# jordisr/poreover

Hardware: AMD Instinct MI355X
Metric: decoded Mbases/s + read-pairs/s, 10k synthetic pairs T~4000, 1/2/4/8 MI355X (higher is better)
Workload: dtype f64; 1 GPU; pair-decode (Viterbi x2 + banded NW + envelope + pair beam row_col) of ONE job of 10000 synthetic pairs, T~4000, C=5, beam_width=5, padding=5; inputs resident in HBM; pairs_per_job=10000, pairs_per_gpu=10000, T=4000, beam_width=5, method=row_col, decoded_pairs_rank0=10000, parallelism=shard1 (no collective)

## Files before the change

poreover_amd/csrc/po_beam2d_pre.h:

```cpp
#pragma once
#include "po_beam2d_common.h"

template <int MODEL>
__global__ __launch_bounds__(64) void beam2d_prepass_kernel(X2Args a) {
    constexpr int K = (MODEL == PO_MODEL_CTC) ? 1 : 3;
    constexpr int nthr = 64;
    const int pi = blockIdx.x, tid = threadIdx.x;
    if (a.use_pre_status && a.status[pi] != PO_OK) {
        if (tid == 0) { a.meta[pi] = make_int2(a.status[pi], -1); a.nmain[pi] = 0; }
        return;
    }
    const int64_t o1 = a.y1_off[pi], o2 = a.y2_off[pi];
    const int64_t b2 = a.y2_off[0];
    const int U = (int)(a.y1_off[pi + 1] - o1), V = (int)(a.y2_off[pi + 1] - o2);
    const int32_t* env = a.env + 2 * o1;
    int* envt = a.envt + 2 * (o2 - b2);
    const int A = a.A, W = a.W;
    int st = PO_OK, R = 32;
    if (U < 1 || V < 1 || U >= (1 << 24) || V >= (1 << 24)) st = PO_E_ARG;
    if (st == PO_OK) {
        int bad = 0, wmax = 0, nonmono = 0;
        const int2* env2 = (const int2*)env;
        for (int u = tid; u < U; u += nthr) {
            const int2 e = env2[u];
            const int lo = e.x, hi = e.y;
            const int2 ep = (u > 0) ? env2[u - 1] : make_int2(0, 0);
            const int ln = (u + 1 < U) ? env2[u + 1].x : V;
            if (lo < hi && (lo < 0 || hi > V)) bad = 1;
            if (lo < 0 || hi > V || (u > 0 && (lo < ep.x || hi < ep.y))) nonmono = 1;
            wmax = max(wmax, hi - lo);
            const int hp = (u > 0) ? ep.y : 0;
            for (int x = max(hp, 0); x < min(hi, V); ++x) envt[2 * x] = u;
            for (int x = max(lo, 0); x < min(ln, V); ++x) envt[2 * x + 1] = u;
        }
        __threadfence_block();
        if (__syncthreads_or(bad)) st = PO_E_ENVELOPE;
        const bool mono = !__syncthreads_or(nonmono);
        if (st == PO_OK && mono) {
            const int lo0 = env[0], hil = env[2 * (U - 1) + 1];
            for (int x = tid; x < V; x += nthr) {
                const int a_ = (x < hil) ? envt[2 * x] : 0x7fffffff, b_ = (x >= lo0) ? envt[2 * x + 1] : -1;
                const int c = (a_ != 0x7fffffff && b_ >= a_) ? b_ - a_ + 1 : 0;
                envt[2 * x] = c ? a_ : -1;
                envt[2 * x + 1] = c ? a_ + c : -1;
                wmax = max(wmax, c);
            }
        } else if (st == PO_OK && !a.need_mono) {
            for (int x = tid; x < V; x += nthr) { envt[2 * x] = 0x7fffffff; envt[2 * x + 1] = 0; }
            __syncthreads();
            for (int u = tid; u < U; u += nthr) {
                const int lo = env[2 * u], hi = env[2 * u + 1];
                for (int x = lo; x < hi; ++x) { atomicMin(&envt[2 * x], u); atomicAdd(&envt[2 * x + 1], 1); }
            }
            __syncthreads();
            for (int x = tid; x < V; x += nthr) {
                const int c = envt[2 * x + 1], f = envt[2 * x];
                envt[2 * x] = c ? f : -1;
                envt[2 * x + 1] = c ? f + c : -1;
                wmax = max(wmax, c);
            }
        }
        if (st == PO_OK) {
#pragma unroll
            for (int off = 32; off >= 1; off >>= 1) wmax = max(wmax, __shfl_xor(wmax, off));
            while (R < wmax + 2) R <<= 1;
            const long long pool_entries = (long long)(a.pool_bytes / (8 * K));
            const long long ng = pool_entries / ((long long)PO_A * 2 * R);
            const long long need = 1 + A + (long long)A * max(W, A) * ((long long)min(U, V) + 1);
            if (need >= (1 << 24)) st = PO_E_NOMEM;
            else if (min((long long)a.ngl, ng) < 8 * max(W, PO_A) || ((a.defer_odd & 1) && (pi & 1)) || (a.need_mono && !mono)) R = X2_DEFERRED;
        }
    }
    if (tid == 0) {
        a.meta[pi] = make_int2(st, R);
        a.nmain[pi] = 0;
        if (st == PO_OK && R == X2_DEFERRED) {
            a.queue[16] = 1;
            if (a.defer_count) atomicAdd(a.defer_count, 1ull);
        }
    }
}

__global__ __launch_bounds__(64) void beam2d_walk_kernel(X2Args a) {
    const int pi = blockIdx.x, lane = threadIdx.x;
    const int2 mt = a.meta[pi];
    if (mt.x != PO_OK || mt.y < 0) return;
    const int64_t o1 = a.y1_off[pi], o2 = a.y2_off[pi], b2 = a.y2_off[0];
    const int U = (int)(a.y1_off[pi + 1] - o1), V = (int)(a.y2_off[pi + 1] - o2);
    const int2* env2 = (const int2*)(a.env + 2 * o1);
    const int2* envt2 = (const int2*)(a.envt + 2 * (o2 - b2));
    int4* sc = a.sched + (o2 - b2);
    int u = 0, v = 0, m = 0, werr = 0, ubase = -1000, vbase = -1000;
    int2 erc = make_int2(0, 0), ecc = make_int2(0, 0);
    while (u <= U - 1 && v <= V - 1) {
        if (u < ubase || u >= ubase + 64) { ubase = u; erc = (ubase + lane < U) ? env2[ubase + lane] : make_int2(0, 0); }
        if (v < vbase || v >= vbase + 64) { vbase = v; ecc = (vbase + lane < V) ? envt2[vbase + lane] : make_int2(0, 0); }
        const int ul = u + lane, vl = v + lane;
        const int iu = ul - ubase, iv = vl - vbase;
        const bool have = iu < 64 && iv < 64 && ul < U && vl < V;
        const int ers = __shfl(erc.x, iu & 63), ere = __shfl(erc.y, iu & 63);
        const int ecs = __shfl(ecc.x, iv & 63), ece = __shfl(ecc.y, iv & 63);
        const bool row_ok = (vl >= ers && vl < ere), col_ok = (ul >= ecs && ul < ece);
        const unsigned long long okb = __ballot(have && row_ok && col_ok);
        const unsigned long long haveb = __ballot(have);
        const int run = (~okb == 0ull) ? 64 : __builtin_ctzll(~okb);
        if (lane < run) sc[m + lane] = make_int4(ul, vl, ece, ere);
        m += run; u += run; v += run;
        if (run < 64 && ((haveb >> run) & 1ull)) {
            const unsigned long long c1 = __ballot(!row_ok && vl < ers), c0 = __ballot(!col_ok && ul < ecs);
            if ((c1 >> run) & 1ull) v = __builtin_amdgcn_readlane(ers, run);
            else if ((c0 >> run) & 1ull) {
                const int cs = __builtin_amdgcn_readlane(ecs, run);
                const int rw = u + 1 + lane, ir = rw - ubase;
                const int rws = __shfl(erc.x, ir & 63);
                const unsigned long long same = __ballot(ir < 64 && rw < cs && rw < U && !(v < rws));
                u += 1 + ((~same == 0ull) ? 64 : __builtin_ctzll(~same));
            } else { werr = 1; break; }
        }
    }
    if (lane == 0) {
        a.nmain[pi] = m;
        if (werr) a.meta[pi] = make_int2(PO_E_ENVELOPE, mt.y);
    }
}
```

poreover_amd/csrc/po_pair.hip:

```cpp
#include <algorithm>
#include <atomic>
#include <cstdlib>
#include <type_traits>

#define PO_WANT_ZERO_KERNEL 1
#include "po_device.h"
#include "po_host.h"

namespace {

constexpr int NW_MATCH = 2, NW_MISMATCH = -1, NW_GAP = -1, NW_BAND = 500;
constexpr int SK_PER = 8, SK_BW = SK_PER * 64, SK_MAXB = 256, SK_SEG = 1024;

struct PPArgs {
    const int64_t* y1_off; const int64_t* y2_off;
    int n;
    const char* seq1d; const int64_t* seq1d_off;
    const int32_t* len1; const int32_t* len2;
    const int32_t* map1; const int32_t* map2;
    const int32_t* st1; const int32_t* st2;
    int padding, full_alignment, diagonal_envelope, diagonal_width;
    int band;
    int match, mismatch, gap;
    long long seq_lds_cap;
// ... 480 lines not shown
        }
        }
        if (a.mode == 1) {
            const int64_t ao = a.aln_off[pi];
            const int capo = (int)(a.aln_off[pi + 1] - ao);
            if (ncol > capo) { if (tid == 0) { a.status[pi] = PO_E_CAP; *a.cap_flag = 1; a.ncol_out[pi] = 0; } continue; }
            for (int k = tid; k < ncol; k += NT) { a.aln_out1[ao + k] = al1[ncol - 1 - k]; a.aln_out2[ao + k] = al2[ncol - 1 - k]; }
            if (tid == 0) { a.ncol_out[pi] = ncol; a.status[pi] = PO_OK; }
            continue;
        }
        int matches = 0;
        for (int k = tid; k < ncol; k += NT) matches += (al1[k] == al2[k]);
        int tot_m;
        (void)block_excl_sum(matches, &tot_m);
        const double identity = (double)tot_m / (double)ncol;
        if (a.mode == 0 && identity < 0.5) {
            if (tid == 0) { a.status[pi] = PO_SKIP_IDENTITY; a.identity[pi] = identity; }
            continue;
        }

        PPTK(2);
        if constexpr (SKEW) if (a.maps_increasing) {
            int* const blo = r_start;
            int* const bhi = r_start + a.row_cap + 8;
            int xbase = -1, ybase = -1;
            for (int k0 = 0; k0 < ncol; k0 += PO_WAVE) {
                const int k = k0 + lane;
                const bool in = k < ncol;
                const char ca = in ? al1[ncol - 1 - k] : '-', cb = in ? al2[ncol - 1 - k] : '-';
                const char cn = (k + 1 < ncol) ? al1[ncol - 2 - k] : '-';
                int tx, ty;
                const int ex = block_excl_sum(ca != '-' ? 1 : 0, &tx);
                const int ey = block_excl_sum(cb != '-' ? 1 : 0, &ty);
                if (in) {
                    const int xi = xbase + ex + (ca != '-' ? 1 : 0);
                    const int yi = ybase + ey + (cb != '-' ? 1 : 0);
                    const int i1 = min(max(xi, 0), l1 - 1), i2 = min(max(yi, 0), l2 - 1);
                    const int i1p = min(max(xi - (ca != '-' ? 1 : 0), 0), l1 - 1);
                    const int i1n = min(max(xi + (cn != '-' ? 1 : 0), 0), l1 - 1);
                    if (k == 0 || i1p != i1) blo[i1] = m2[i2];
                    if (k == ncol - 1 || i1n != i1) bhi[i1] = (i2 + 1 < l2) ? m2[i2 + 1] : V;
                }
                xbase += tx;
                ybase += ty;
            }
            psync();
            {
                const int f0 = min(m1[0], U);
                int lo = 0, hi = min(V, -1 + a.padding);
                if (lo > hi) lo = 0;
                for (int u = lane; u < f0; u += PO_WAVE) { env[2 * u] = lo; env[2 * u + 1] = hi; }
            }
            int pe_ = 0;
            for (int b0 = 0; b0 < l1; b0 += PO_WAVE) {
                const int b = b0 + lane;
                const bool in = b < l1;
                int lo = 0, hi = 0, r0 = 0, r1 = 0;
                if (in) {
                    lo = max(0, blo[b] - a.padding);
                    hi = min(V, bhi[b] + a.padding);
                    if (lo > hi) lo = 0;
                    r0 = m1[b];
                    r1 = min((b + 1 < l1) ? m1[b + 1] : U, U);
                }
                int lo_first = lo, pos = 0;
                for (;;) {
                    const unsigned long long mk = __ballot(in && r0 < r1 && lane >= pos && lo_first > pe_);
                    if (mk == 0ull) break;
                    const int qs = __builtin_ctzll(mk);
                    if (lane == qs) lo_first = pe_;
                    pe_ = __builtin_amdgcn_readlane(hi, qs);
                    pos = qs + 1;
                }
                for (int u = r0; u < r1; ++u) { env[2 * u] = (u == r0) ? lo_first : lo; env[2 * u + 1] = hi; }
            }
            if (tid == 0) { a.status[pi] = PO_OK; if (a.identity) a.identity[pi] = identity; }
            PPTK(3);
#ifdef PO_PP_TIMING
            if (tid == 0 && pi == 0) printf("[pp timing] pair 0: setup %lld fill %lld traceback %lld envelope %lld ticks (10 ns)\n", tk_[0], tk_[1], tk_[2], tk_[3]);
#endif
            continue;
        }
        for (int u = tid; u < U; u += NT) { env[2 * u] = INT_MAX; env[2 * u + 1] = -1; }
        __syncthreads();
        int xbase = -1, ybase = -1;
        for (int k0 = 0; k0 < ncol; k0 += NT) {
            const int k = k0 + tid;
            const bool in = k < ncol;
            const char ca = in ? al1[ncol - 1 - k] : '-', cb = in ? al2[ncol - 1 - k] : '-';
            int tx, ty;
            const int ex = block_excl_sum(ca != '-' ? 1 : 0, &tx);
            const int ey = block_excl_sum(cb != '-' ? 1 : 0, &ty);
            if (in) {
                const int xi = xbase + ex + (ca != '-' ? 1 : 0);
                const int yi = ybase + ey + (cb != '-' ? 1 : 0);
                const int i1 = min(max(xi, 0), l1 - 1), i2 = min(max(yi, 0), l2 - 1);
                const int sx = m1[i1], exr = (i1 + 1 < l1) ? m1[i1 + 1] : U;
                const int sy = m2[i2], eyr = (i2 + 1 < l2) ? m2[i2 + 1] : V;
                for (int i = sx; i < exr; ++i)
                    if (i < U) { atomicMin(&env[2 * i], sy); atomicMax(&env[2 * i + 1], eyr); }
            }
            xbase += tx;
            ybase += ty;
        }
        __threadfence_block();
        __syncthreads();
        int prev_end = 0;
        for (int u0 = 0; u0 < U; u0 += NT) {
            const int u = u0 + tid;
            if (u < U) {
                int lo = env[2 * u], hi = env[2 * u + 1];
                if (lo == INT_MAX) lo = -1;
                lo = max(0, lo - a.padding);
                hi = min(V, hi + a.padding);
                lo_s[tid] = lo; hi_s[tid] = hi;
            }
            __syncthreads();
            if (tid < PO_WAVE) {
                const int cnt = min(NT, U - u0);
                int pe_ = prev_end;
                for (int b0 = 0; b0 < cnt; b0 += PO_WAVE) {
                    const int q = b0 + lane;
                    const bool in = q < cnt;
                    int lo = in ? lo_s[q] : 0;
                    const int hi = in ? hi_s[q] : 0;
                    if (lo > hi) lo = 0;
                    int pos = 0;
                    for (;;) {
                        const unsigned long long mk = __ballot(in && lane >= pos && lo > pe_);
                        if (mk == 0ull) break;
                        const int qs = __builtin_ctzll(mk);
                        if (lane == qs) lo = pe_;
                        pe_ = __builtin_amdgcn_readlane(hi, qs);
                        pos = qs + 1;
                    }
                    if (in) lo_s[q] = lo;
                }
                if (lane == 0) sh[4] = pe_;
            }
            __syncthreads();
            prev_end = sh[4];
            if (u < U) { env[2 * u] = lo_s[tid]; env[2 * u + 1] = hi_s[tid]; }
            __syncthreads();
        }
        if (tid == 0) { a.status[pi] = PO_OK; if (a.identity) a.identity[pi] = identity; }
        PPTK(3);
#ifdef PO_PP_TIMING
        if (tid == 0 && pi == 0) printf("[pp timing] pair 0: setup %lld fill %lld traceback %lld envelope %lld ticks (10 ns)\n", tk_[0], tk_[1], tk_[2], tk_[3]);
#endif
    }
}

extern "C" {
int po_launch_viterbi_strided(const double*, const int64_t*, int, int, int, uint32_t, int, int8_t*, char*,
                              const int64_t*, int, int, int32_t*, int32_t*, int32_t*, int8_t*, int8_t*, hipStream_t);
size_t po_beam2d_ws_bytes_impl(int, int64_t, int64_t, int64_t, int64_t, int, int, int, int);
int po_launch_beam2d_geom(const double*, const int64_t*, const double*, const int64_t*, const int32_t*, int, int, int,
                          uint32_t, int, int, int, int64_t, int64_t, int64_t, int64_t, char*, const int64_t*, int32_t*, int32_t*,
                          int, void*, size_t, hipStream_t);
void po_prof_stage(int kernel, hipStream_t s, int begin, void** tok);
}

static std::atomic<int> g_pp_legacy{-1};
extern "C" int po_set_align_route(int legacy) {
    g_pp_legacy.store(legacy ? 1 : 0);
    return PO_OK;
}
static bool pp_legacy() {
    int v = g_pp_legacy.load();
    if (v < 0) {
        const char* e = getenv("PO_PP_LEGACY");
        v = (e != nullptr && atoi(e) != 0) ? 1 : 0;
        g_pp_legacy.store(v);
    }
    return v != 0;
}

namespace {
void pp_launch(PPArgs a, int blocks, int one_wave, hipStream_t stream, long long max_len2 = 0) {
    long long cap = (a.mode == 2) ? 0 : ((a.row_cap + 15) & ~15LL);
    if (cap > 24 * 1024) cap = 0;
    a.seq_lds_cap = cap;
    const size_t lds = (size_t)(2 * cap);
    const bool legacy = pp_legacy();
    const bool skew = one_wave && !a.full_alignment && a.mode != 2 && !legacy && max_len2 <= (long long)SK_MAXB * SK_BW;
    if (skew) hipLaunchKernelGGL((pair_prep_kernel<64, true>), dim3(blocks), dim3(64), lds, stream, a);
    else if (one_wave) hipLaunchKernelGGL((pair_prep_kernel<64, false>), dim3(blocks), dim3(64), lds, stream, a);
    else hipLaunchKernelGGL((pair_prep_kernel<256, false>), dim3(blocks), dim3(256), lds, stream, a);
}
}

namespace {
inline size_t al256(size_t b) { return (b + 255) & ~size_t(255); }

inline size_t pp_skew_cells(int64_t l1, int64_t l2, int64_t band) {
    const int64_t nb = l2 / SK_BW + 1;
    const int64_t rows = 2 * (l1 + 1) + ((l1 + 1) * (2 * band + 1) + l2) / SK_BW + 1 + nb;
    return (size_t)(64 * (rows + 63 * nb));
}

struct PPGeom {
    int blocks, one_wave;
    size_t dp_cap, row_cap, aln_cap;
    int big_blocks;
    size_t big_dp_cap, big_row_cap, big_aln_cap, off_big_dp, off_big_rows, off_big_aln;
    size_t off_queue, off_map1, off_map2, off_st1, off_st2, off_dp, off_rows, off_aln, off_ff, off_env, off_b2, total;
    size_t ff_bytes, b2_bytes;
};

size_t pp_total_mem() { return po_dev_info().mem; }

int pp_num_cus() { return po_dev_info().cus; }

PPGeom pp_geometry(int n, int64_t tr1, int64_t tr2, int64_t mr1, int64_t mr2, int C, const po_pair_options* opt) {
    PPGeom g;
    g.one_wave = opt->full_alignment ? 0 : 1;
    g.blocks = std::min(n > 0 ? n : 1, pp_num_cus() * (g.one_wave ? 16 : 4));
    const int64_t lmax1 = std::max<int64_t>(64, mr1 / 4 + 8), lmax2 = std::max<int64_t>(64, mr2 / 4 + 8);
    g.row_cap = (size_t)(lmax1 + 1);
    const int64_t width = opt->full_alignment ? (lmax2 + 1) : std::min<int64_t>(lmax2 + 1, 2 * NW_BAND + 1);
    const bool skew_only = g.one_wave && !pp_legacy() && lmax2 <= (int64_t)SK_MAXB * SK_BW && mr2 + 8 <= (int64_t)SK_MAXB * SK_BW;
    g.dp_cap = skew_only ? pp_skew_cells(lmax1, lmax2, NW_BAND) : (size_t)((lmax1 + 1) * width);
    if (g.one_wave && !skew_only) g.dp_cap = std::max(g.dp_cap, pp_skew_cells(lmax1, lmax2, NW_BAND));
    g.aln_cap = (size_t)(lmax1 + lmax2 + 16);
    {
        static const size_t budget = [] { const char* e = getenv("PO_PP_BUDGET_MB"); return (size_t)(e ? atoi(e) : 5120) << 20; }();
        const size_t per_block = sizeof(int) * g.dp_cap + sizeof(int) * 4 * g.row_cap + 2 * g.aln_cap;
        const size_t pb = std::max<size_t>(per_block, 1);
        const size_t fit_budget = std::max<size_t>(budget / pb, (size_t)pp_num_cus());
        const size_t fit_mem = std::max<size_t>(1, (pp_total_mem() / 16) / pb);
        g.blocks = (int)std::min<size_t>((size_t)g.blocks, std::max<size_t>(1, std::min(fit_budget, fit_mem)));
    }
    {
        const int64_t b1 = mr1 + 8, b2 = mr2 + 8;
        g.big_row_cap = (size_t)(b1 + 1);
        const int64_t bw = opt->full_alignment ? (b2 + 1) : std::min<int64_t>(b2 + 1, 2 * NW_BAND + 1);
        g.big_dp_cap = skew_only ? pp_skew_cells(b1, b2, NW_BAND) : (size_t)((b1 + 1) * bw);
        if (g.one_wave && !skew_only) g.big_dp_cap = std::max(g.big_dp_cap, pp_skew_cells(b1, b2, NW_BAND));
        g.big_aln_cap = (size_t)(b1 + b2 + 16);
        const size_t per_block = sizeof(int) * g.big_dp_cap + sizeof(int) * 4 * g.big_row_cap + 2 * g.big_aln_cap;
        const size_t fit = ((size_t)2 << 30) / std::max<size_t>(per_block, 1);
        g.big_blocks = (int)std::max<size_t>(1, std::min<size_t>(std::min<size_t>(32, fit), (size_t)(n > 0 ? n : 1)));
        if (per_block > pp_total_mem() / 8) g.big_blocks = 0;
    }
    const int kind = opt->model == PO_MODEL_FLIPFLOP ? PO_KIND_FLIPFLOP : PO_KIND_POREOVER;
    g.ff_bytes = (kind == PO_KIND_FLIPFLOP) ? al256((size_t)std::max(tr1, tr2) * 8) + al256((size_t)std::max(tr1, tr2)) : 0;
    g.b2_bytes = po_beam2d_ws_bytes_impl(n, tr1, tr2, mr1, mr2, C, opt->beam_width, opt->model, opt->method);
    size_t o = 0;
    g.off_queue = o; o += 256;
    g.off_map1 = o; o += al256(sizeof(int32_t) * (size_t)tr1);
    g.off_map2 = o; o += al256(sizeof(int32_t) * (size_t)tr2);
    g.off_st1 = o; o += al256(sizeof(int32_t) * (size_t)n);
    g.off_st2 = o; o += al256(sizeof(int32_t) * (size_t)n);
    g.off_dp = o; o += al256(sizeof(int) * g.dp_cap * g.blocks);
    g.off_rows = o; o += al256(sizeof(int) * 4 * g.row_cap * g.blocks);
    g.off_aln = o; o += al256(2 * g.aln_cap * g.blocks);
    g.off_big_dp = o; o += al256(sizeof(int) * g.big_dp_cap * g.big_blocks);
    g.off_big_rows = o; o += al256(sizeof(int) * 4 * g.big_row_cap * g.big_blocks);
    g.off_big_aln = o; o += al256(2 * g.big_aln_cap * g.big_blocks);
    g.off_ff = o; o += g.ff_bytes;
    g.off_env = o; o += al256(sizeof(int32_t) * 2 * (size_t)tr1);
    g.off_b2 = o; o += g.b2_bytes;
    g.total = o + 256;
    return g;
}
}

extern "C" size_t po_pair_ws_bytes_impl(int n, int64_t tr1, int64_t tr2, int64_t mr1, int64_t mr2, int C,
                                        const po_pair_options* opt) {
    return pp_geometry(n, tr1, tr2, mr1, mr2, C, opt).total;
}

extern "C" int po_launch_pair_decode_geom(const double* y1, const int64_t* y1_off, const double* y2,
                                          const int64_t* y2_off, int n, int C, const po_pair_options* opt,
                                          int64_t tr1, int64_t tr2, int64_t mr1, int64_t mr2,
                                          const int32_t* ext_map1, const int32_t* ext_map2, char* seq1d,
                                          const int64_t* seq1d_off, int32_t* len1, int32_t* len2, double* identity,
                                          int32_t* env_out, char* seq, const int64_t* seq_off, int32_t* seq_len,
                                          int32_t* status, void* ws, size_t ws_bytes, hipStream_t stream) {
    if (n <= 0) return PO_OK;
    const int A = PO_A;
    const uint32_t alphabet = 'A' | ('C' << 8) | ('G' << 16) | ((uint32_t)'T' << 24);
    if (opt->model < 0 || opt->model > 2) return PO_E_ARG;
    if ((opt->model == PO_MODEL_FLIPFLOP) ? (C != 2 * A) : (C != A + 1)) return PO_E_ARG;
    const int kind = opt->model == PO_MODEL_CTC ? PO_KIND_POREOVER
                                                 : (opt->model == PO_MODEL_MERGE ? PO_KIND_BONITO : PO_KIND_FLIPFLOP);
    const PPGeom g = pp_geometry(n, tr1, tr2, mr1, mr2, C, opt);
    if (ws_bytes < g.total) return PO_E_CAP;
    char* w = (char*)ws;
    int32_t* map1 = (int32_t*)(w + g.off_map1);
    int32_t* map2 = (int32_t*)(w + g.off_map2);
    int32_t* st1 = (int32_t*)(w + g.off_st1);
    int32_t* st2 = (int32_t*)(w + g.off_st2);
    int32_t* env = env_out ? env_out : (int32_t*)(w + g.off_env);
    int8_t* ffp = g.ff_bytes ? (int8_t*)(w + g.off_ff) : nullptr;
    int8_t* ffpath = ffp ? ffp + al256((size_t)std::max(tr1, tr2) * 8) : nullptr;
    void* tok = nullptr;
    int rc;
    if (ext_map1 && ext_map2) {
        map1 = const_cast<int32_t*>(ext_map1);
        map2 = const_cast<int32_t*>(ext_map2);
        if (po_zero_async(st1, sizeof(int32_t) * n, stream) != hipSuccess) return PO_E_HIP;
        if (po_zero_async(st2, sizeof(int32_t) * n, stream) != hipSuccess) return PO_E_HIP;
    } else if (!opt->diagonal_envelope) {
        po_prof_stage(PO_K_VITERBI, stream, 1, &tok);
        rc = po_launch_viterbi_strided(y1, y1_off, n, C, A, alphabet, kind, nullptr, seq1d, seq1d_off, 0, 2, len1, map1,
                                       st1, ffp, ffpath, stream);
        if (rc != PO_OK) return rc;
        rc = po_launch_viterbi_strided(y2, y2_off, n, C, A, alphabet, kind, nullptr, seq1d, seq1d_off, 1, 2, len2, map2,
                                       st2, ffp, ffpath, stream);
        if (rc != PO_OK) return rc;
        po_prof_stage(PO_K_VITERBI, stream, 0, &tok);
    } else {
        if (po_zero_async(len1, sizeof(int32_t) * n, stream) != hipSuccess) return PO_E_HIP;
        if (po_zero_async(len2, sizeof(int32_t) * n, stream) != hipSuccess) return PO_E_HIP;
    }
    PPArgs a;
    a.y1_off = y1_off; a.y2_off = y2_off; a.n = n;
    a.seq1d = seq1d; a.seq1d_off = seq1d_off; a.len1 = len1; a.len2 = len2;
    a.map1 = map1; a.map2 = map2; a.st1 = st1; a.st2 = st2;
    a.padding = opt->padding; a.full_alignment = opt->full_alignment;
    a.diagonal_envelope = opt->diagonal_envelope; a.diagonal_width = opt->diagonal_width;
    a.band = NW_BAND; a.mode = 0; a.retry_cap = 0;
    a.maps_increasing = (ext_map1 && ext_map2) ? 0 : 1;
    a.match = NW_MATCH; a.mismatch = NW_MISMATCH; a.gap = NW_GAP;
    a.lenU = a.lenV = nullptr; a.map1_off = a.map2_off = nullptr; a.aln_out1 = a.aln_out2 = nullptr;
    a.aln_off = nullptr; a.ncol_out = nullptr; a.env_off = nullptr;
    a.env = env; a.identity = identity; a.status = status;
    a.queue = (int*)(w + g.off_queue);
    a.cap_flag = a.queue + 32;
    a.dp = (int*)(w + g.off_dp); a.dp_cap = (long long)g.dp_cap;
    a.rowinfo = (int*)(w + g.off_rows); a.row_cap = (long long)g.row_cap;
    a.aln = w + g.off_aln; a.aln_cap = (long long)g.aln_cap;
    if (po_zero_async(a.queue, 256, stream) != hipSuccess) return PO_E_HIP;
    po_prof_stage(PO_K_ALIGN, stream, 1, &tok);
    pp_launch(a, g.blocks, g.one_wave, stream, mr2 + 8);
    if (g.big_blocks > 0 && !opt->diagonal_envelope) {
        PPArgs b = a;
        b.retry_cap = 1;
        b.queue = a.queue + 16;
        b.dp = (int*)(w + g.off_big_dp); b.dp_cap = (long long)g.big_dp_cap;
        b.rowinfo = (int*)(w + g.off_big_rows); b.row_cap = (long long)g.big_row_cap;
        b.aln = w + g.off_big_aln; b.aln_cap = (long long)g.big_aln_cap;
        pp_launch(b, g.big_blocks, g.one_wave, stream, mr2 + 8);
    }
    po_prof_stage(PO_K_ALIGN, stream, 0, &tok);
    po_prof_stage(PO_K_BEAM2D, stream, 1, &tok);
    rc = po_launch_beam2d_geom(y1, y1_off, y2, y2_off, env, n, C, A, alphabet, opt->beam_width, opt->model, opt->method,
                               tr1, tr2, mr1, mr2, seq, seq_off, seq_len, status, 1, w + g.off_b2, g.b2_bytes, stream);
    po_prof_stage(PO_K_BEAM2D, stream, 0, &tok);
    return rc;
}

extern "C" int po_launch_pair_decode(const double* y1, const int64_t* y1_off, const double* y2, const int64_t* y2_off,
                                     int n, int C, const po_pair_options* opt, char* seq1d, const int64_t* seq1d_off,
                                     int32_t* len1, int32_t* len2, double* identity, int32_t* env_out, char* seq,
                                     const int64_t* seq_off, int32_t* seq_len, int32_t* status, void* ws,
                                     size_t ws_bytes, hipStream_t stream) {
    if (n <= 0) return PO_OK;
    int64_t* h = (int64_t*)malloc(sizeof(int64_t) * 2 * (size_t)(n + 1));
    if (!h) return PO_E_NOMEM;
    int rc = PO_OK;
    if (hipMemcpyAsync(h, y1_off, sizeof(int64_t) * (n + 1), hipMemcpyDeviceToHost, stream) != hipSuccess ||
        hipMemcpyAsync(h + n + 1, y2_off, sizeof(int64_t) * (n + 1), hipMemcpyDeviceToHost, stream) != hipSuccess ||
        hipStreamSynchronize(stream) != hipSuccess)
        rc = PO_E_HIP;
    int64_t m1 = 0, m2 = 0, t1 = 0, t2 = 0;
    if (rc == PO_OK) {
        for (int i = 0; i < n; ++i) {
            m1 = std::max<int64_t>(m1, h[i + 1] - h[i]);
            m2 = std::max<int64_t>(m2, h[n + 1 + i + 1] - h[n + 1 + i]);
        }
        t1 = h[n] - h[0];
        t2 = h[2 * n + 1] - h[n + 1];
    }
    free(h);
    if (rc != PO_OK) return rc;
    return po_launch_pair_decode_geom(y1, y1_off, y2, y2_off, n, C, opt, t1, t2, m1, m2, nullptr, nullptr, seq1d, seq1d_off, len1, len2,
                                      identity, env_out, seq, seq_off, seq_len, status, ws, ws_bytes, stream);
}

extern "C" size_t po_align_ws_bytes(int n, int64_t max_len1, int64_t max_len2, int band) {
    const int blocks = std::min(n > 0 ? n : 1, pp_num_cus() * 4);
    const int64_t width = band > 0 ? std::min<int64_t>(max_len2 + 1, 2 * (int64_t)band + 1) : max_len2 + 1;
    size_t cells = (size_t)((max_len1 + 1) * width);
    if (band > 0) cells = std::max(cells, pp_skew_cells(max_len1, max_len2, band));
    return 256 + al256(sizeof(int) * cells * blocks) + al256(sizeof(int) * 4 * (size_t)(max_len1 + 2) * blocks) +
           al256(2 * (size_t)(max_len1 + max_len2 + 16) * blocks) + 256;
}

extern "C" int po_launch_align_scores(const char* seqs, const int64_t* seq_off, int n, int band, int match, int mismatch,
                                      int gap, int64_t max_len1, int64_t max_len2, char* aln1, char* aln2,
                                      const int64_t* aln_off, int32_t* ncol, int32_t* status, void* ws, size_t ws_bytes,
                                      hipStream_t stream);
extern "C" int po_launch_align(const char* seqs, const int64_t* seq_off, int n, int band, int64_t max_len1,
                               int64_t max_len2, char* aln1, char* aln2, const int64_t* aln_off, int32_t* ncol,
                               int32_t* status, void* ws, size_t ws_bytes, hipStream_t stream) {
    return po_launch_align_scores(seqs, seq_off, n, band, NW_MATCH, NW_MISMATCH, NW_GAP, max_len1, max_len2, aln1, aln2, aln_off,
                                  ncol, status, ws, ws_bytes, stream);
}
extern "C" int po_launch_align_scores(const char* seqs, const int64_t* seq_off, int n, int band, int match, int mismatch,
                                      int gap, int64_t max_len1, int64_t max_len2, char* aln1, char* aln2,
                                      const int64_t* aln_off, int32_t* ncol, int32_t* status, void* ws, size_t ws_bytes,
                                      hipStream_t stream) {
    if (n <= 0) return PO_OK;
    if (ws_bytes < po_align_ws_bytes(n, max_len1, max_len2, band)) return PO_E_CAP;
    const int blocks = std::min(n, pp_num_cus() * 4);
    const int64_t width = band > 0 ? std::min<int64_t>(max_len2 + 1, 2 * (int64_t)band + 1) : max_len2 + 1;
    char* w = (char*)ws;
    const int one_wave = band > 0 ? 1 : 0;
    PPArgs a = {};
    a.n = n; a.seq1d = seqs; a.seq1d_off = seq_off; a.mode = 1;
    a.full_alignment = band > 0 ? 0 : 1; a.band = band > 0 ? band : 0;
    a.match = match; a.mismatch = mismatch; a.gap = gap;
    a.aln_out1 = aln1; a.aln_out2 = aln2; a.aln_off = aln_off; a.ncol_out = ncol; a.status = status;
    size_t o = 0;
    a.queue = (int*)(w + o); o += 256;
    a.cap_flag = a.queue + 32;
    a.dp_cap = (long long)((max_len1 + 1) * width);
    if (band > 0) a.dp_cap = std::max<long long>(a.dp_cap, (long long)pp_skew_cells(max_len1, max_len2, band));
    a.dp = (int*)(w + o); o += al256(sizeof(int) * (size_t)a.dp_cap * blocks);
    a.row_cap = (long long)(max_len1 + 2); a.rowinfo = (int*)(w + o); o += al256(sizeof(int) * 4 * (size_t)a.row_cap * blocks);
    a.aln_cap = (long long)(max_len1 + max_len2 + 16); a.aln = w + o;
    if (po_zero_async(a.queue, 256, stream) != hipSuccess) return PO_E_HIP;
    pp_launch(a, blocks, one_wave, stream, max_len2);
    return PO_OK;
}

__global__ __launch_bounds__(64) void nw_matrix_kernel(const char* seqs, const int64_t* seq_off, int n, int match, int mismatch, int gap,
                                                       int32_t* dp, const int64_t* dp_off, int32_t* status) {
    const int p = (int)blockIdx.x, lane = (int)threadIdx.x;
    if (p >= n) return;
    const char* const s1 = seqs + seq_off[2 * p];
    const char* const s2 = seqs + seq_off[2 * p + 1];
    const int l1 = (int)(seq_off[2 * p + 1] - seq_off[2 * p]), l2 = (int)(seq_off[2 * p + 2] - seq_off[2 * p + 1]);
    int32_t* const M = dp + dp_off[p];
    const int64_t Wd = (int64_t)l2 + 1;
    for (int j = lane; j <= l2; j += 64) M[j] = gap * j;
    for (int i = 1; i <= l1; ++i) {
        po_wave_sync();
        const int32_t* const up_ = M + (int64_t)(i - 1) * Wd;
        int32_t* const row = M + (int64_t)i * Wd;
        const char ci = s1[i - 1];
        int carry = gap * i;
        if (lane == 0) row[0] = carry;
        for (int base = 1; base <= l2; base += 64) {
            const int j = base + lane;
            const bool ok = j <= l2;
            int v = INT_MIN / 2;
            if (ok) {
                const int sc = (ci == s2[j - 1]) ? match : mismatch;
                v = max(up_[j - 1] + sc, up_[j] + gap) - gap * j;
            }
#pragma unroll
            for (int d = 1; d < 64; d <<= 1) {
                const int o = __shfl_up(v, d);
                if (lane >= d) v = max(v, o);
            }
            v = max(v, carry);
            if (ok) row[j] = v + gap * j;
            carry = __shfl(v, 63);
        }
    }
// ... 52 lines not shown
```

poreover_amd/csrc/po_viterbi.hip:

```cpp
#include <cstdlib>

#include "po_device.h"

#define VT_THREADS 256
#define VT_WAVES (VT_THREADS / PO_WAVE)

__device__ __forceinline__ int block_exclusive_count(bool flag, int* wsum, int* total) {
    const unsigned long long mask = __ballot(flag);
    const int lane = po_lane(), wave = threadIdx.x >> 6;
    const int below = __popcll(mask & ((1ull << lane) - 1ull));
    if (lane == 0) wsum[wave] = __popcll(mask);
    __syncthreads();
    int base = 0, tot = 0;
#pragma unroll
    for (int w = 0; w < VT_WAVES; ++w) {
        const int c = wsum[w];
        if (w < wave) base += c;
        tot += c;
    }
    __syncthreads();
    *total = tot;
    return base + below;
}

#define VT_FPT 2
#define VT_CMAX (PO_A + 1)
template <int THREADS>
__global__ __launch_bounds__(THREADS) void viterbi_ctc_kernel(
    const double* __restrict__ y, const int64_t* __restrict__ y_off, int C, uint32_t alphabet, int kind,
    int8_t* __restrict__ path, char* __restrict__ seq, const int64_t* __restrict__ seq_off, int so_base,
    int so_stride, int32_t* __restrict__ seq_len, int32_t* __restrict__ map, int32_t* __restrict__ status) {
    constexpr int VT_WAVES_ = THREADS / PO_WAVE, VT_TILE = THREADS * VT_FPT, VT_LD = (VT_TILE * VT_CMAX) / THREADS;
    __shared__ double tile[VT_TILE * VT_CMAX];
    __shared__ int wsum[VT_WAVES_];
    __shared__ int8_t pth[VT_TILE + 1];
    const int r = blockIdx.x, tid = threadIdx.x;
    const int64_t r0 = y_off[r];
    const int T = (int)(y_off[r + 1] - r0);
    const int blank = C - 1;
    const double* yr = y + r0 * C;
    const int64_t so = seq_off[so_base + (int64_t)r * so_stride];
    char* sq = seq + so;
    const int cap = (int)(seq_off[so_base + (int64_t)r * so_stride + 1] - so);
    int32_t* mp = map ? map + r0 : nullptr;
    int n_seq = 0, n_map = 0, st = PO_OK;

    int last_state = -1;
    if (kind == PO_KIND_BONITO && T > 0) {
        const double* row = yr + (int64_t)(T - 1) * C;
        int b = 0;
        double bv = row[0];
        for (int c = 1; c < C; ++c) {
            const double v = row[c];
            if (v > bv) { bv = v; b = c; }
        }
        last_state = b;
    }
    if (tid == 0) pth[0] = -1;
    __syncthreads();

    for (int t0 = 0; t0 < T; t0 += VT_TILE) {
        const int rows = min(VT_TILE, T - t0);
        const int nval = rows * C;
        const double* src = yr + (int64_t)t0 * C;
        double2 reg[VT_LD / 2];
        const double2* src2 = (const double2*)src;
        const int nval2 = nval >> 1;
#pragma unroll
        for (int q = 0; q < VT_LD / 2; ++q) {
            const int i = tid + q * THREADS;
            reg[q] = (i < nval2) ? src2[i] : make_double2(0.0, 0.0);
        }
        const double tail = (nval & 1) ? src[nval - 1] : 0.0;
#pragma unroll
        for (int q = 0; q < VT_LD / 2; ++q) {
            const int i = tid + q * THREADS;
            if (i < nval2) { tile[2 * i] = reg[q].x; tile[2 * i + 1] = reg[q].y; }
        }
        if ((nval & 1) && tid == 0) tile[nval - 1] = tail;
        __syncthreads();
        int p[VT_FPT];
#pragma unroll
        for (int f = 0; f < VT_FPT; ++f) {
            const int fr = tid * VT_FPT + f;
            p[f] = blank;
            if (fr < rows) {
                double bv = tile[fr * C];
                int b = 0;
                for (int c = 1; c < C; ++c) {
                    const double v = tile[fr * C + c];
                    if (v > bv) { bv = v; b = c; }
                }
                p[f] = b;
                pth[fr + 1] = (int8_t)b;
                if (path) path[r0 + t0 + fr] = (int8_t)b;
            }
        }
        __syncthreads();
        bool emit[VT_FPT], emit_map[VT_FPT];
        int ne = 0, nm = 0;
#pragma unroll
        for (int f = 0; f < VT_FPT; ++f) {
            const int fr = tid * VT_FPT + f, t = t0 + fr;
            const int prev = pth[fr];
            emit[f] = emit_map[f] = false;
            if (fr < rows && p[f] != blank) {
                if (kind == PO_KIND_POREOVER) {
                    emit[f] = emit_map[f] = true;
                } else {
                    emit[f] = (t == 0) || (p[f] != prev);
                    emit_map[f] = (p[f] != ((t == 0) ? last_state : prev));
                }
            }
            ne += emit[f];
            nm += emit_map[f];
        }
        auto block_excl = [&](int v, int* total) {
            const int lane = po_lane(), wave = tid >> 6;
            int inc = v;
#pragma unroll
            for (int o = 1; o < PO_WAVE; o <<= 1) {
                const int t = __shfl_up(inc, o);
                if (lane >= o) inc += t;
            }
            if (lane == PO_WAVE - 1) wsum[wave] = inc;
            __syncthreads();
            int base = 0, tot = 0;
#pragma unroll
            for (int w = 0; w < VT_WAVES_; ++w) {
                const int c = wsum[w];
                if (w < wave) base += c;
                tot += c;
            }
            __syncthreads();
            *total = tot;
            return base + inc - v;
        };
        int tot_p;
        const int excl = block_excl(ne | (nm << 16), &tot_p);
        int pos_s = n_seq + (excl & 0xffff);
#pragma unroll
        for (int f = 0; f < VT_FPT; ++f)
            if (emit[f]) {
                if (pos_s < cap) sq[pos_s] = (char)((alphabet >> (8 * p[f])) & 0xffu);
                else st = PO_E_CAP;
                pos_s++;
            }
        n_seq += tot_p & 0xffff;
        if (mp) {
            int pos_m = n_map + (excl >> 16);
#pragma unroll
            for (int f = 0; f < VT_FPT; ++f)
                if (emit_map[f]) mp[pos_m++] = t0 + tid * VT_FPT + f;
            n_map += tot_p >> 16;
        }
        if (tid == 0) pth[0] = pth[rows];
        __syncthreads();
    }
    if (__syncthreads_or(st != PO_OK)) st = PO_E_CAP;
    if (st == PO_OK && mp && n_map != n_seq) st = PO_E_ARG;
    if (T < 1) st = PO_E_ARG;
    if (tid == 0) {
        seq_len[r] = n_seq;
        status[r] = st;
    }
}

#define FF_S 8
__global__ __launch_bounds__(PO_WAVE) void flipflop_dp_kernel(const double* __restrict__ y,
                                                              const int64_t* __restrict__ y_off, int n, int A,
                                                              int8_t* __restrict__ ptr,
                                                              int8_t* __restrict__ path,
                                                              int32_t* __restrict__ status) {
    __shared__ __attribute__((aligned(8))) int8_t chunk[8][512 * FF_S];
    const int lane = po_lane(), g = lane >> 3, j = lane & 7;
    const int r = blockIdx.x * 8 + g;
    const bool live = r < n;
    const int64_t r0 = live ? y_off[r] : 0;
    const int T = live ? (int)(y_off[r + 1] - r0) : 0;
    int Tmax = T;
#pragma unroll
    for (int o = 8; o < PO_WAVE; o <<= 1) Tmax = max(Tmax, __shfl_xor(Tmax, o));
    const int S = 2 * A;
    const double* yr = y + r0 * S;
    int8_t* pr = ptr + r0 * FF_S;
    double v = (T > 0 && j < S) ? yr[j] : PO_NEG_INF;
    constexpr int FF_PF = 16;
    auto row_at = [&](int t) -> double { return (t < T && j < S) ? yr[(int64_t)t * S + j] : 0.0; };
    double yq[FF_PF];
    int bq[FF_PF];
#pragma unroll
    for (int i = 0; i < FF_PF; ++i) { yq[i] = row_at(1 + i); bq[i] = -1; }
    for (int t0 = 1; t0 < Tmax + FF_PF; t0 += FF_PF) {
#pragma unroll
        for (int i = 0; i < FF_PF; ++i) po_settle(yq[i]);
        double yn[FF_PF];
#pragma unroll
        for (int i = 0; i < FF_PF; ++i) yn[i] = row_at(t0 + FF_PF + i);
#pragma unroll
        for (int i = 0; i < FF_PF; ++i)
            if (bq[i] >= 0) pr[(int64_t)(t0 - FF_PF + i) * FF_S + j] = (int8_t)bq[i];
#pragma unroll
        for (int f = 0; f < FF_PF; ++f) {
            const int t = t0 + f;
            bq[f] = -1;
            if (t < Tmax) {
                const bool on = t < T;
                const double yt = yq[f];
                double bv = 0;
                int bi = 0;
#pragma unroll
                for (int i = 0; i < FF_S; ++i) {
                    const double vi = __shfl(v, (g << 3) | i);
                    const double tr = (j < A) ? 1.0 : (((i % A) == (j - A)) ? 1.0 : 0.0);
                    const double cand = tr + vi;
                    if (i < S && (i == 0 || cand > bv)) { bv = cand; bi = i; }
                }
                if (on && j < S) {
                    bq[f] = bi;
                    v = yt + bv;
                }
            }
        }
#pragma unroll
        for (int i = 0; i < FF_PF; ++i) yq[i] = yn[i];
    }
    double bv = __shfl(v, g << 3);
    int best = 0;
#pragma unroll
    for (int i = 1; i < FF_S; ++i) {
        const double vi = __shfl(v, (g << 3) | i);
        if (i < S && vi > bv) { bv = vi; best = i; }
    }
    __threadfence_block();
    int cur = best;
    for (int lo = ((Tmax + 511) / 512 - 1) * 512; lo >= 0; lo -= 512) {
        const int hi = min(T, lo + 512), len = hi - lo;
        {
            const unsigned long long* src = (const unsigned long long*)(pr + (int64_t)lo * FF_S);
            unsigned long long* dst = (unsigned long long*)&chunk[g][0];
            if (((unsigned long long)src & 7ull) == 0ull) {
                for (int f = j; f < len; f += 8) dst[f] = src[f];
            } else {
                for (int i = j; i < len * FF_S; i += 8) chunk[g][i] = pr[(int64_t)lo * FF_S + i];
            }
        }
        __syncthreads();
        if (j == 0) {
            for (int t = hi - 1; t >= lo; --t) {
                path[r0 + t] = (int8_t)cur;
                if (t > 0) cur = chunk[g][(t - lo) * FF_S + cur];
            }
        }
        cur = __shfl(cur, g << 3);
        __syncthreads();
    }
    if (live && j == 0) status[r] = (T < 1) ? PO_E_ARG : PO_OK;
}

__global__ __launch_bounds__(VT_THREADS) void flipflop_compact_kernel(
    const int8_t* __restrict__ path, const int64_t* __restrict__ y_off, int A, uint32_t alphabet,
    char* __restrict__ seq, const int64_t* __restrict__ seq_off, int so_base, int so_stride,
    int32_t* __restrict__ seq_len, int32_t* __restrict__ map, int32_t* __restrict__ status) {
    __shared__ int wsum[VT_WAVES];
    const int r = blockIdx.x, tid = threadIdx.x;
    const int64_t r0 = y_off[r];
    const int T = (int)(y_off[r + 1] - r0);
    const int64_t so = seq_off[so_base + (int64_t)r * so_stride];
    char* sq = seq + so;
    const int cap = (int)(seq_off[so_base + (int64_t)r * so_stride + 1] - so);
    int n_seq = 0, st = PO_OK;
    for (int t0 = 0; t0 < T; t0 += VT_THREADS) {
        const int t = t0 + tid;
        bool emit = false;
        int p = 0;
        if (t < T) {
            p = path[r0 + t];
            emit = (t == 0) || (p != path[r0 + t - 1]);
        }
        int tot;
        const int pos = n_seq + block_exclusive_count(emit, wsum, &tot);
        if (emit) {
            if (pos < cap) {
                sq[pos] = (char)((alphabet >> (8 * (p % A))) & 0xffu);
                if (map) map[r0 + pos] = t;
            } else st = PO_E_CAP;
        }
        n_seq += tot;
    }
    if (__syncthreads_or(st != PO_OK)) st = PO_E_CAP;
    if (tid == 0) {
        seq_len[r] = n_seq;
        if (status[r] == PO_OK) status[r] = st;
    }
}

extern "C" int po_launch_viterbi_strided(const double* y, const int64_t* y_off, int n, int C, int A,
                                         uint32_t alphabet, int kind, int8_t* path, char* seq,
                                         const int64_t* seq_off, int so_base, int so_stride, int32_t* seq_len,
                                         int32_t* map, int32_t* status, int8_t* ff_ptr, int8_t* ff_path,
                                         hipStream_t stream);

extern "C" int po_launch_viterbi(const double* y, const int64_t* y_off, int n, int C, int A, uint32_t alphabet,
                                 int kind, int8_t* path, char* seq, const int64_t* seq_off, int32_t* seq_len,
                                 int32_t* map, int32_t* status, int8_t* ff_ptr, int8_t* ff_path,
                                 hipStream_t stream) {
    return po_launch_viterbi_strided(y, y_off, n, C, A, alphabet, kind, path, seq, seq_off, 0, 1, seq_len, map,
                                     status, ff_ptr, ff_path, stream);
}

extern "C" int po_launch_viterbi_strided(const double* y, const int64_t* y_off, int n, int C, int A,
                                         uint32_t alphabet, int kind, int8_t* path, char* seq,
                                         const int64_t* seq_off, int so_base, int so_stride, int32_t* seq_len,
                                         int32_t* map, int32_t* status, int8_t* ff_ptr, int8_t* ff_path,
                                         hipStream_t stream) {
    if (n <= 0) return PO_OK;
    if (A < 1 || A > PO_A) return PO_E_ARG;
    if (kind == PO_KIND_FLIPFLOP) {
        if (C != 2 * A) return PO_E_ARG;
        int8_t* pth = path ? path : ff_path;
        hipLaunchKernelGGL(flipflop_dp_kernel, dim3((n + 7) / 8), dim3(PO_WAVE), 0, stream, y, y_off, n, A, ff_ptr,
                           pth, status);
        hipLaunchKernelGGL(flipflop_compact_kernel, dim3(n), dim3(VT_THREADS), 0, stream, pth, y_off, A, alphabet,
                           seq, seq_off, so_base, so_stride, seq_len, map, status);
        return PO_OK;
    }
    if (kind != PO_KIND_POREOVER && kind != PO_KIND_BONITO) return PO_E_ARG;
    if (C != A + 1) return PO_E_ARG;
    static const int vt_threads = [] { const char* e = getenv("PO_VT_THREADS"); return (e && atoi(e) == 256) ? 256 : 64; }();
    if (vt_threads == 256)
        hipLaunchKernelGGL(viterbi_ctc_kernel<256>, dim3(n), dim3(256), 0, stream, y, y_off, C, alphabet, kind, path, seq,
                           seq_off, so_base, so_stride, seq_len, map, status);
    else
        hipLaunchKernelGGL(viterbi_ctc_kernel<64>, dim3(n), dim3(64), 0, stream, y, y_off, C, alphabet, kind, path, seq,
                           seq_off, so_base, so_stride, seq_len, map, status);
    return PO_OK;
}
```

Before: 190,400 read-pairs/s.

## Batch envelope prepass loads, widen walk window, fuse paired Viterbi launches with prefetch

```diff
diff --git a/poreover_amd/csrc/po_beam2d_pre.h b/poreover_amd/csrc/po_beam2d_pre.h
--- a/poreover_amd/csrc/po_beam2d_pre.h
+++ b/poreover_amd/csrc/po_beam2d_pre.h
@@ -1,6 +1,7 @@
 #pragma once
 #include "po_beam2d_common.h"
 
+#define PRE_NB 8
 template <int MODEL>
 __global__ __launch_bounds__(64) void beam2d_prepass_kernel(X2Args a) {
     constexpr int K = (MODEL == PO_MODEL_CTC) ? 1 : 3;
@@ -21,29 +22,59 @@
     if (st == PO_OK) {
         int bad = 0, wmax = 0, nonmono = 0;
         const int2* env2 = (const int2*)env;
-        for (int u = tid; u < U; u += nthr) {
-            const int2 e = env2[u];
-            const int lo = e.x, hi = e.y;
-            const int2 ep = (u > 0) ? env2[u - 1] : make_int2(0, 0);
-            const int ln = (u + 1 < U) ? env2[u + 1].x : V;
-            if (lo < hi && (lo < 0 || hi > V)) bad = 1;
-            if (lo < 0 || hi > V || (u > 0 && (lo < ep.x || hi < ep.y))) nonmono = 1;
-            wmax = max(wmax, hi - lo);
-            const int hp = (u > 0) ? ep.y : 0;
-            for (int x = max(hp, 0); x < min(hi, V); ++x) envt[2 * x] = u;
-            for (int x = max(lo, 0); x < min(ln, V); ++x) envt[2 * x + 1] = u;
+        int2* envt2 = (int2*)envt;
+        const int lo0 = env[0], hil = env[2 * (U - 1) + 1];
+        int2 carry = make_int2(0, 0);
+        for (int u0 = 0; u0 < U; u0 += nthr * PRE_NB) {
+            int2 e[PRE_NB];
+#pragma unroll
+            for (int k = 0; k < PRE_NB; ++k) {
+                const int u = u0 + k * nthr + tid;
+                e[k] = (u < U) ? env2[u] : make_int2(V, V);
+            }
+            const int un = u0 + nthr * PRE_NB;
+            const int lnext = (un < U) ? env2[un].x : V;
+#pragma unroll
+            for (int k = 0; k < PRE_NB; ++k) {
+                const int u = u0 + k * nthr + tid;
+                const int lo = e[k].x, hi = e[k].y;
+                const int px = __shfl(e[k].x, (tid + 63) & 63), py = __shfl(e[k].y, (tid + 63) & 63), nx = __shfl(e[k].x, (tid + 1) & 63);
+                const int2 last = (k == 0) ? carry : make_int2(__shfl(e[k > 0 ? k - 1 : 0].x, 63), __shfl(e[k > 0 ? k - 1 : 0].y, 63));
+                const int first = (k + 1 < PRE_NB) ? __shfl(e[k + 1 < PRE_NB ? k + 1 : k].x, 0) : lnext;
+                const int2 ep = (tid == 0) ? last : make_int2(px, py);
+                const int ln = (tid == 63) ? first : nx;
+                if (u < U) {
+                    if (lo < hi && (lo < 0 || hi > V)) bad = 1;
+                    if (lo < 0 || hi > V || (u > 0 && (lo < ep.x || hi < ep.y))) nonmono = 1;
+                    wmax = max(wmax, hi - lo);
+                    const int hp = (u > 0) ? ep.y : 0;
+                    for (int x = max(hp, 0); x < min(hi, V); ++x) envt[2 * x] = u;
+                    for (int x = max(lo, 0); x < min(ln, V); ++x) envt[2 * x + 1] = u;
+                }
+            }
+            carry = make_int2(__shfl(e[PRE_NB - 1].x, 63), __shfl(e[PRE_NB - 1].y, 63));
         }
         __threadfence_block();
         if (__syncthreads_or(bad)) st = PO_E_ENVELOPE;
         const bool mono = !__syncthreads_or(nonmono);
         if (st == PO_OK && mono) {
-            const int lo0 = env[0], hil = env[2 * (U - 1) + 1];
-            for (int x = tid; x < V; x += nthr) {
-                const int a_ = (x < hil) ? envt[2 * x] : 0x7fffffff, b_ = (x >= lo0) ? envt[2 * x + 1] : -1;
-                const int c = (a_ != 0x7fffffff && b_ >= a_) ? b_ - a_ + 1 : 0;
-                envt[2 * x] = c ? a_ : -1;
-                envt[2 * x + 1] = c ? a_ + c : -1;
-                wmax = max(wmax, c);
+            for (int x0 = 0; x0 < V; x0 += nthr * PRE_NB) {
+                int2 c2[PRE_NB];
+#pragma unroll
+                for (int k = 0; k < PRE_NB; ++k) {
+                    const int x = x0 + k * nthr + tid;
+                    c2[k] = (x < V) ? envt2[x] : make_int2(0, 0);
+                }
+#pragma unroll
+                for (int k = 0; k < PRE_NB; ++k) {
+                    const int x = x0 + k * nthr + tid;
+                    if (x < V) {
+                        const int a_ = (x < hil) ? c2[k].x : 0x7fffffff, b_ = (x >= lo0) ? c2[k].y : -1;
+                        const int c = (a_ != 0x7fffffff && b_ >= a_) ? b_ - a_ + 1 : 0;
+                        envt2[x] = make_int2(c ? a_ : -1, c ? a_ + c : -1);
+                        wmax = max(wmax, c);
+                    }
+                }
             }
         } else if (st == PO_OK && !a.need_mono) {
             for (int x = tid; x < V; x += nthr) { envt[2 * x] = 0x7fffffff; envt[2 * x + 1] = 0; }
@@ -81,6 +112,31 @@
     }
 }
 
+#define WK_NB 4
+struct WalkWin {
+    int2 r0, r1, r2, r3;
+    int base;
+};
+__device__ __forceinline__ void walk_fill(WalkWin& w, const int2* src, int pos, int n, int lane) {
+    w.base = pos;
+    const int p = pos + lane;
+    w.r0 = (p < n) ? src[p] : make_int2(0, 0);
+    w.r1 = (p + 64 < n) ? src[p + 64] : make_int2(0, 0);
+    w.r2 = (p + 128 < n) ? src[p + 128] : make_int2(0, 0);
+    w.r3 = (p + 192 < n) ? src[p + 192] : make_int2(0, 0);
+}
+__device__ __forceinline__ void walk_settle(WalkWin& w) {
+    po_settle(w.r0.x, w.r0.y); po_settle(w.r1.x, w.r1.y); po_settle(w.r2.x, w.r2.y); po_settle(w.r3.x, w.r3.y);
+}
+__device__ __forceinline__ int2 walk_rot(const WalkWin& w, int off, int lane) {
+    const int j0 = off >> 6, s = off & 63;
+    const int2 v0 = w.r0, v1 = w.r1, v2 = w.r2, v3 = w.r3;
+    const int lox = (j0 == 0) ? v0.x : (j0 == 1) ? v1.x : (j0 == 2) ? v2.x : v3.x;
+    const int loy = (j0 == 0) ? v0.y : (j0 == 1) ? v1.y : (j0 == 2) ? v2.y : v3.y;
+    const int hix = (j0 == 0) ? v1.x : (j0 == 1) ? v2.x : v3.x;
+    const int hiy = (j0 == 0) ? v1.y : (j0 == 1) ? v2.y : v3.y;
+    return (lane >= s) ? make_int2(lox, loy) : make_int2(hix, hiy);
+}
 __global__ __launch_bounds__(64) void beam2d_walk_kernel(X2Args a) {
     const int pi = blockIdx.x, lane = threadIdx.x;
     const int2 mt = a.meta[pi];
@@ -90,16 +146,25 @@
     const int2* env2 = (const int2*)(a.env + 2 * o1);
     const int2* envt2 = (const int2*)(a.envt + 2 * (o2 - b2));
     int4* sc = a.sched + (o2 - b2);
-    int u = 0, v = 0, m = 0, werr = 0, ubase = -1000, vbase = -1000;
-    int2 erc = make_int2(0, 0), ecc = make_int2(0, 0);
+    constexpr int WK_REACH = (WK_NB - 1) * 64;
+    int u = 0, v = 0, m = 0, werr = 0;
+    WalkWin wr, wc;
+    walk_fill(wr, env2, 0, U, lane);
+    walk_fill(wc, envt2, 0, V, lane);
+    walk_settle(wr); walk_settle(wc);
     while (u <= U - 1 && v <= V - 1) {
-        if (u < ubase || u >= ubase + 64) { ubase = u; erc = (ubase + lane < U) ? env2[ubase + lane] : make_int2(0, 0); }
-        if (v < vbase || v >= vbase + 64) { vbase = v; ecc = (vbase + lane < V) ? envt2[vbase + lane] : make_int2(0, 0); }
+        const bool fr = u < wr.base || u >= wr.base + WK_REACH, fc = v < wc.base || v >= wc.base + WK_REACH;
+        if (fr || fc) {
+            if (fr) walk_fill(wr, env2, u, U, lane);
+            if (fc) walk_fill(wc, envt2, v, V, lane);
+            walk_settle(wr); walk_settle(wc);
+        }
         const int ul = u + lane, vl = v + lane;
-        const int iu = ul - ubase, iv = vl - vbase;
-        const bool have = iu < 64 && iv < 64 && ul < U && vl < V;
-        const int ers = __shfl(erc.x, iu & 63), ere = __shfl(erc.y, iu & 63);
-        const int ecs = __shfl(ecc.x, iv & 63), ece = __shfl(ecc.y, iv & 63);
+        const int su = (u - wr.base + lane) & 63, sv = (v - wc.base + lane) & 63;
+        const bool have = ul < U && vl < V;
+        const int2 er = walk_rot(wr, u - wr.base, lane), ec = walk_rot(wc, v - wc.base, lane);
+        const int ers = __shfl(er.x, su), ere = __shfl(er.y, su);
+        const int ecs = __shfl(ec.x, sv), ece = __shfl(ec.y, sv);
         const bool row_ok = (vl >= ers && vl < ere), col_ok = (ul >= ecs && ul < ece);
         const unsigned long long okb = __ballot(have && row_ok && col_ok);
         const unsigned long long haveb = __ballot(have);
@@ -111,9 +176,11 @@
             if ((c1 >> run) & 1ull) v = __builtin_amdgcn_readlane(ers, run);
             else if ((c0 >> run) & 1ull) {
                 const int cs = __builtin_amdgcn_readlane(ecs, run);
-                const int rw = u + 1 + lane, ir = rw - ubase;
-                const int rws = __shfl(erc.x, ir & 63);
-                const unsigned long long same = __ballot(ir < 64 && rw < cs && rw < U && !(v < rws));
+                const int rw = u + 1 + lane;
+                const int orw = u + 1 - wr.base;
+                const int2 e1 = walk_rot(wr, orw, lane);
+                const int rws = __shfl(e1.x, (orw + lane) & 63);
+                const unsigned long long same = __ballot(orw + lane < WK_NB * 64 && rw < cs && rw < U && !(v < rws));
                 u += 1 + ((~same == 0ull) ? 64 : __builtin_ctzll(~same));
             } else { werr = 1; break; }
         }
diff --git a/poreover_amd/csrc/po_pair.hip b/poreover_amd/csrc/po_pair.hip
--- a/poreover_amd/csrc/po_pair.hip
+++ b/poreover_amd/csrc/po_pair.hip
@@ -656,8 +656,8 @@
 }
 
 extern "C" {
-int po_launch_viterbi_strided(const double*, const int64_t*, int, int, int, uint32_t, int, int8_t*, char*,
-                              const int64_t*, int, int, int32_t*, int32_t*, int32_t*, int8_t*, int8_t*, hipStream_t);
+int po_launch_viterbi_pair(const double*, const int64_t*, const double*, const int64_t*, int, int, int, uint32_t, int, char*,
+                           const int64_t*, int32_t*, int32_t*, int32_t*, int32_t*, int32_t*, int32_t*, int8_t*, int8_t*, hipStream_t);
 size_t po_beam2d_ws_bytes_impl(int, int64_t, int64_t, int64_t, int64_t, int, int, int, int);
 int po_launch_beam2d_geom(const double*, const int64_t*, const double*, const int64_t*, const int32_t*, int, int, int,
                           uint32_t, int, int, int, int64_t, int64_t, int64_t, int64_t, char*, const int64_t*, int32_t*, int32_t*,
@@ -808,11 +808,8 @@
         if (po_zero_async(st2, sizeof(int32_t) * n, stream) != hipSuccess) return PO_E_HIP;
     } else if (!opt->diagonal_envelope) {
         po_prof_stage(PO_K_VITERBI, stream, 1, &tok);
-        rc = po_launch_viterbi_strided(y1, y1_off, n, C, A, alphabet, kind, nullptr, seq1d, seq1d_off, 0, 2, len1, map1,
-                                       st1, ffp, ffpath, stream);
-        if (rc != PO_OK) return rc;
-        rc = po_launch_viterbi_strided(y2, y2_off, n, C, A, alphabet, kind, nullptr, seq1d, seq1d_off, 1, 2, len2, map2,
-                                       st2, ffp, ffpath, stream);
+        rc = po_launch_viterbi_pair(y1, y1_off, y2, y2_off, n, C, A, alphabet, kind, seq1d, seq1d_off, len1, len2, map1, map2,
+                                    st1, st2, ffp, ffpath, stream);
         if (rc != PO_OK) return rc;
         po_prof_stage(PO_K_VITERBI, stream, 0, &tok);
     } else {
diff --git a/poreover_amd/csrc/po_viterbi.hip b/poreover_amd/csrc/po_viterbi.hip
--- a/poreover_amd/csrc/po_viterbi.hip
+++ b/poreover_amd/csrc/po_viterbi.hip
@@ -26,15 +26,15 @@
 #define VT_FPT 2
 #define VT_CMAX (PO_A + 1)
 template <int THREADS>
-__global__ __launch_bounds__(THREADS) void viterbi_ctc_kernel(
-    const double* __restrict__ y, const int64_t* __restrict__ y_off, int C, uint32_t alphabet, int kind,
+__device__ __forceinline__ void viterbi_ctc_read(
+    const int r, const double* __restrict__ y, const int64_t* __restrict__ y_off, int C, uint32_t alphabet, int kind,
     int8_t* __restrict__ path, char* __restrict__ seq, const int64_t* __restrict__ seq_off, int so_base,
     int so_stride, int32_t* __restrict__ seq_len, int32_t* __restrict__ map, int32_t* __restrict__ status) {
     constexpr int VT_WAVES_ = THREADS / PO_WAVE, VT_TILE = THREADS * VT_FPT, VT_LD = (VT_TILE * VT_CMAX) / THREADS;
     __shared__ double tile[VT_TILE * VT_CMAX];
     __shared__ int wsum[VT_WAVES_];
     __shared__ int8_t pth[VT_TILE + 1];
-    const int r = blockIdx.x, tid = threadIdx.x;
+    const int tid = threadIdx.x;
     const int64_t r0 = y_off[r];
     const int T = (int)(y_off[r + 1] - r0);
     const int blank = C - 1;
@@ -59,25 +59,32 @@
     if (tid == 0) pth[0] = -1;
     __syncthreads();
 
+    double2 reg[VT_LD / 2];
+    double tail = 0.0;
+    auto request = [&](int t0) {
+        const int nval = min(VT_TILE, T - t0) * C;
+        const double* src = yr + (int64_t)t0 * C;
+        const double2* src2 = (const double2*)src;
+        const int nval2 = nval >> 1;
+#pragma unroll
+        for (int q = 0; q < VT_LD / 2; ++q) {
+            const int i = tid + q * THREADS;
+            reg[q] = (i < nval2) ? src2[i] : make_double2(0.0, 0.0);
+        }
+        tail = (nval > 0 && (nval & 1)) ? src[nval - 1] : 0.0;
+    };
+    request(0);
     for (int t0 = 0; t0 < T; t0 += VT_TILE) {
         const int rows = min(VT_TILE, T - t0);
         const int nval = rows * C;
-        const double* src = yr + (int64_t)t0 * C;
-        double2 reg[VT_LD / 2];
-        const double2* src2 = (const double2*)src;
         const int nval2 = nval >> 1;
-#pragma unroll
-        for (int q = 0; q < VT_LD / 2; ++q) {
-            const int i = tid + q * THREADS;
-            reg[q] = (i < nval2) ? src2[i] : make_double2(0.0, 0.0);
-        }
-        const double tail = (nval & 1) ? src[nval - 1] : 0.0;
 #pragma unroll
         for (int q = 0; q < VT_LD / 2; ++q) {
             const int i = tid + q * THREADS;
             if (i < nval2) { tile[2 * i] = reg[q].x; tile[2 * i + 1] = reg[q].y; }
         }
         if ((nval & 1) && tid == 0) tile[nval - 1] = tail;
+        request(t0 + VT_TILE);
         __syncthreads();
         int p[VT_FPT];
 #pragma unroll
@@ -164,6 +171,34 @@
         seq_len[r] = n_seq;
         status[r] = st;
     }
+}
+
+template <int THREADS>
+__global__ __launch_bounds__(THREADS) void viterbi_ctc_kernel(
+    const double* __restrict__ y, const int64_t* __restrict__ y_off, int C, uint32_t alphabet, int kind,
+    int8_t* __restrict__ path, char* __restrict__ seq, const int64_t* __restrict__ seq_off, int so_base,
+    int so_stride, int32_t* __restrict__ seq_len, int32_t* __restrict__ map, int32_t* __restrict__ status) {
+    viterbi_ctc_read<THREADS>(blockIdx.x, y, y_off, C, alphabet, kind, path, seq, seq_off, so_base, so_stride, seq_len, map, status);
+}
+
+struct VtPairArgs {
+    const double* y[2];
+    const int64_t* y_off[2];
+    int32_t* seq_len[2];
+    int32_t* map[2];
+    int32_t* status[2];
+    char* seq;
+    const int64_t* seq_off;
+    int n, C, kind;
+    uint32_t alphabet;
+};
+template <int THREADS>
+__global__ __launch_bounds__(THREADS) void viterbi_ctc_pair_kernel(VtPairArgs a) {
+    const int which = ((int)blockIdx.x >= a.n) ? 1 : 0;
+    const int r = (int)blockIdx.x - which * a.n;
+    viterbi_ctc_read<THREADS>(r, which ? a.y[1] : a.y[0], which ? a.y_off[1] : a.y_off[0], a.C, a.alphabet, a.kind, nullptr, a.seq,
+                              a.seq_off, which, 2, which ? a.seq_len[1] : a.seq_len[0], which ? a.map[1] : a.map[0],
+                              which ? a.status[1] : a.status[0]);
 }
 
 #define FF_S 8
@@ -336,3 +371,28 @@
                            seq_off, so_base, so_stride, seq_len, map, status);
     return PO_OK;
 }
+
+extern "C" int po_launch_viterbi_pair(const double* y1, const int64_t* y1_off, const double* y2, const int64_t* y2_off, int n,
+                                      int C, int A, uint32_t alphabet, int kind, char* seq, const int64_t* seq_off,
+                                      int32_t* len1, int32_t* len2, int32_t* map1, int32_t* map2, int32_t* st1,
+                                      int32_t* st2, int8_t* ff_ptr, int8_t* ff_path, hipStream_t stream) {
+    if (n <= 0) return PO_OK;
+    static const bool split = [] { const char* e = getenv("PO_VT_SPLIT"); return e && atoi(e) != 0; }();
+    static const bool four_waves = [] { const char* e = getenv("PO_VT_THREADS"); return e && atoi(e) == 256; }();
+    if (kind == PO_KIND_FLIPFLOP || split || four_waves || n > (1 << 30)) {
+        const int rc = po_launch_viterbi_strided(y1, y1_off, n, C, A, alphabet, kind, nullptr, seq, seq_off, 0, 2, len1, map1, st1,
+                                                 ff_ptr, ff_path, stream);
+        if (rc != PO_OK) return rc;
+        return po_launch_viterbi_strided(y2, y2_off, n, C, A, alphabet, kind, nullptr, seq, seq_off, 1, 2, len2, map2, st2, ff_ptr,
+                                         ff_path, stream);
+    }
+    if (A < 1 || A > PO_A) return PO_E_ARG;
+    if (kind != PO_KIND_POREOVER && kind != PO_KIND_BONITO) return PO_E_ARG;
+    if (C != A + 1) return PO_E_ARG;
+    VtPairArgs a;
+    a.y[0] = y1; a.y[1] = y2; a.y_off[0] = y1_off; a.y_off[1] = y2_off;
+    a.seq_len[0] = len1; a.seq_len[1] = len2; a.map[0] = map1; a.map[1] = map2; a.status[0] = st1; a.status[1] = st2;
+    a.seq = seq; a.seq_off = seq_off; a.n = n; a.C = C; a.kind = kind; a.alphabet = alphabet;
+    hipLaunchKernelGGL(viterbi_ctc_pair_kernel<64>, dim3(2 * (unsigned)n), dim3(64), 0, stream, a);
+    return PO_OK;
+}
```

Result: no change. 191,100 read-pairs/s (median of 6 runs) (+0.4%).
